# matthewygf/Tiresias

Hardware: AMD Instinct MI355X
Metric: avg JCT + makespan on NSDI'19 Microsoft trace, 8×MI355X cluster (lower is better)
Workload: dtype bf16

## Files before the change

### csrc/bindings/ops.cpp

```cpp
#include <array>
#include <ATen/ATen.h>
#include <c10/hip/HIPStream.h>
#include <torch/library.h>

#include <functional>
#include <map>
#include <mutex>
#include <sstream>
#include <tuple>
#include <vector>

#include "tam/kernels.h"
#include "tam/launch.h"
#include "tam/gemm8p.h"

using at::Tensor;
using c10::optional;

namespace {

hipStream_t cur_stream(const Tensor& t) {
  return c10::hip::getCurrentHIPStream(t.device().index()).stream();
}

// ... 708 lines not shown

void bn_backward_op(const Tensor& dy, const optional<Tensor>& y, const Tensor& x, const Tensor& mean,
                    const Tensor& rstd, const Tensor& gamma, const Tensor& dx,
                    const optional<Tensor>& dres, const optional<Tensor>& dgamma,
                    const optional<Tensor>& dbeta, bool relu, const optional<Tensor>& addend,
                    const optional<Tensor>& sums, bool sums_ready, const optional<Tensor>& ymask) {
  check_bf16(dy, "dy"); check_bf16(x, "x"); check_bf16(dx, "dx");
  check_contig(dy, "dy"); check_contig(x, "x"); check_contig(dx, "dx");
  const int64_t C = x.size(-1);
  const int64_t M = x.numel() / C;
  TORCH_CHECK(C % 8 == 0 && C <= 2048, "tam.bn: C must be a multiple of 8 and <= 2048");
  const bool has_mask = ymask.has_value() && ymask->defined();
  TORCH_CHECK(!relu || (y.has_value() && y->defined()) || has_mask, "tam.bn_backward: relu needs y or ymask");
  if (has_mask)
    TORCH_CHECK(ymask->is_cuda() && ymask->scalar_type() == at::kByte && ymask->is_contiguous() &&
                ymask->numel() == x.numel() / 8, "tam.bn_backward: ymask must be uint8 [numel/8]");
  const tam::bf16_t* yp = has_mask ? nullptr : opt_ptr<const tam::bf16_t>(y);
  const bool has_add = addend.has_value() && addend->defined();
  if (has_add) {
    check_bf16(*addend, "addend"); check_contig(*addend, "addend");
    TORCH_CHECK(addend->numel() == dy.numel(), "tam.bn_backward: addend size");
  }
  TORCH_CHECK(!sums_ready || ((sums.has_value() && sums->defined()) && !relu && !has_add &&
                              !(dres.has_value() && dres->defined())),
              "tam.bn_backward: sums_ready takes the already-masked gradient (no relu / addend / dres)");
  Tensor tmp;
  double* sp = bn_sums(sums, x, C, tmp, "tam.bn_backward");
  tam::bn_backward(bp(dy), opt_ptr<const tam::bf16_t>(addend), yp, bp(x), mean.data_ptr<float>(),
                   rstd.data_ptr<float>(), gamma.data_ptr<float>(), M, (int)C, relu, bpm(dx),
                   opt_ptr<tam::bf16_t>(dres), opt_ptr<float>(dgamma), opt_ptr<float>(dbeta),
                   sp, sums_ready ? 1 : 0, has_mask ? ymask->data_ptr<uint8_t>() : nullptr, cur_stream(x));
}

static tam::LnDrop drop_args(const optional<Tensor>& rec, int64_t site, int64_t thr, double scale,
                             const Tensor& like, const char* op) {
  tam::LnDrop d;
  if (!(rec.has_value() && rec->defined())) return d;
  TORCH_CHECK(rec->scalar_type() == at::kInt && rec->numel() >= 4 && rec->is_contiguous() &&
                  rec->device() == like.device(),
              op, ": drop_rec must be an int32 [4] tensor on the data's device");
  TORCH_CHECK(thr > 0 && thr < 65536 && site >= 0 && site <= 0x7fffffff, op, ": drop_thr in (0, 65536), drop_site >= 0");
  d.rec = rec->data_ptr<int>();
  d.site = (unsigned)site;
  d.thr = (unsigned)thr;
  d.scale = (float)scale;
  return d;
}

void ln_forward_op(const Tensor& x, const Tensor& g, const Tensor& b, const Tensor& y,
                   const Tensor& mean, const Tensor& rstd, double eps, const optional<Tensor>& addend,
                   const optional<Tensor>& sum_out, const optional<Tensor>& drop_rec, int64_t drop_site,
                   int64_t drop_thr, double drop_scale) {
  check_bf16(x, "x"); check_bf16(y, "y"); check_contig(x, "x"); check_contig(y, "y");
  check_f32(g, "g"); check_f32(b, "b");
  const int64_t D = x.size(-1);
  TORCH_CHECK(D % 8 == 0 && D <= 2048, "tam.ln: D must be a multiple of 8 and <= 2048");
  const bool add = addend.has_value() && addend->defined();
  TORCH_CHECK(add == (sum_out.has_value() && sum_out->defined()), "tam.ln_forward: addend needs sum_out");
  if (add) {
    check_bf16(*addend, "addend"); check_contig(*addend, "addend");
    check_bf16(*sum_out, "sum_out"); check_contig(*sum_out, "sum_out");
    TORCH_CHECK(addend->numel() == x.numel() && sum_out->numel() == x.numel(), "tam.ln_forward: addend size");
  }
  const tam::LnDrop drop = drop_args(drop_rec, drop_site, drop_thr, drop_scale, x, "tam.ln_forward");
  TORCH_CHECK(!drop.rec || add, "tam.ln_forward: drop_rec needs addend");
  tam::ln_forward(bp(x), g.data_ptr<float>(), b.data_ptr<float>(), bpm(y), mean.data_ptr<float>(),
// ... 561 lines not shown
                 const optional<Tensor>& dc_next, const optional<Tensor>& dgates,
                 const optional<Tensor>& dc_prev, const optional<Tensor>& dgates_bf16) {
  check_f32(act, "act");
  const int B = (int)act.size(0), Hd = (int)(act.size(1) / 5);
  tam::lstm_cell_backward(act.data_ptr<float>(), opt_ptr<const float>(c_prev), nullptr,
                          opt_ptr<const float>(dh), opt_ptr<const float>(dc_next),
                          opt_ptr<float>(dgates), opt_ptr<float>(dc_prev),
                          opt_ptr<tam::bf16_t>(dgates_bf16), B, Hd, c10::hip::getCurrentHIPStream(act.device().index()).stream());
}

}

TORCH_LIBRARY(tam, m) {
  m.def("gemm(Tensor a, bool a_kmajor, Tensor b, bool b_kmajor, Tensor(a!) c, int mode, Tensor? bias, bool relu, Tensor? mask, float alpha, bool allow_split, Tensor(b!)? colsum=None) -> ()", &gemm_op);
  m.def("conv_fwd(Tensor x, Tensor w, Tensor(a!) y, int stride, int pad, int dil, Tensor? bias, bool relu, Tensor(b!)? stats=None) -> int", &conv_fwd_op);
  m.def("conv_dgrad(Tensor dy, Tensor w, Tensor(a!) wt, Tensor(b!) dx, int stride, int pad, int dil, Tensor? mask) -> ()", &conv_dgrad_op);
  m.def("conv_weight_t_batch(Tensor[] w, Tensor(a!)[] wt) -> ()", &conv_weight_t_batch_op);
  m.def("gemm_wgrad_grouped(Tensor[] dy, Tensor[] x, Tensor(a!)[] dw, Tensor(b!)[] db, int[]? modes=None) -> ()", &gemm_wgrad_grouped_op);
  m.def("gemm_wgrad_grouped_ok(int M, int N, int K) -> bool", &gemm_wgrad_grouped_ok_op);
  m.def("gemm_grouped_tile(int tile) -> ()", &gemm_grouped_tile_op);
  m.def("conv_dgrad_pre(Tensor dy, Tensor w, Tensor wt, Tensor(a!) dx, int stride, int pad, int dil, Tensor? mask, Tensor(b!)? stats=None, Tensor? bnx=None, Tensor? bnmean=None, Tensor? bnrstd=None) -> int", &conv_dgrad_pre_op);
  m.def("conv_wgrad(Tensor dy, Tensor x, Tensor(a!) dw, int stride, int pad, int dil, int mode, Tensor(b!)? dbias=None, bool patch=True) -> ()", &conv_wgrad_op);
  m.def("conv_wgrad_deferred(Tensor dy, Tensor x, Tensor(a!) dw, int stride, int pad, int dil, int mode, Tensor(b!)? dbias, bool patch) -> (Tensor, int)", &conv_wgrad_deferred_op);
  m.def("wgrad_slab_reduce_many(Tensor[] slabs, int[] sp, Tensor(a!)[] dw, int[] mode) -> ()", &wgrad_slab_reduce_many_op);
  m.def("bn_forward(Tensor x, Tensor? res, Tensor(a!) y, Tensor gamma, Tensor beta, Tensor(b!)? run_mean, Tensor(c!)? run_var, Tensor(d!) save_mean, Tensor(e!) save_rstd, float eps, float momentum, bool relu, Tensor(f!)? sums=None, bool sums_ready=False, Tensor(g!)? ymask=None) -> ()", &bn_forward_op);
  m.def("bn_backward(Tensor dy, Tensor? y, Tensor x, Tensor mean, Tensor rstd, Tensor gamma, Tensor(a!) dx, Tensor(b!)? dres, Tensor(c!)? dgamma, Tensor(d!)? dbeta, bool relu, Tensor? addend=None, Tensor(e!)? sums=None, bool sums_ready=False, Tensor? ymask=None) -> ()", &bn_backward_op);
  m.def("ln_forward(Tensor x, Tensor g, Tensor b, Tensor(a!) y, Tensor(b!) mean, Tensor(c!) rstd, float eps, Tensor? addend=None, Tensor(d!)? sum_out=None, Tensor? drop_rec=None, int drop_site=0, int drop_thr=0, float drop_scale=1.0) -> ()", &ln_forward_op);
  m.def("ln_backward(Tensor dy, Tensor x, Tensor g, Tensor mean, Tensor rstd, Tensor(a!) dx, Tensor(b!) dg, Tensor(c!) db, Tensor? addend=None, Tensor(d!)? dr=None, Tensor? drop_rec=None, int drop_site=0, int drop_thr=0, float drop_scale=1.0) -> ()", &ln_backward_op);
  m.def("ln_backward_split(Tensor dy, Tensor x, Tensor g, Tensor mean, Tensor rstd, Tensor(a!) dx, Tensor(b!) ws, Tensor? addend=None, Tensor(c!)? dr=None, Tensor? drop_rec=None, int drop_site=0, int drop_thr=0, float drop_scale=1.0) -> int", &ln_backward_split_op);
  m.def("dropout_apply(Tensor x, Tensor(a!) y, Tensor rec, int site, int thr, float scale) -> ()", &dropout_apply_op);
  m.def("dropout_advance(Tensor(a!) rec) -> ()", &dropout_advance_op);
  m.def("col_reduce_acc(Tensor part, int nblk, int W, Tensor(a!) out0, Tensor(b!) out1, int split) -> ()", &col_reduce_acc_op);
  m.def("col_reduce_acc_batch(Tensor[] parts, int[] nblk, Tensor(a!)[] out0, Tensor(b!)[] out1) -> ()", &col_reduce_acc_batch_op);
  m.def("maxpool_forward(Tensor x, Tensor(a!) y, Tensor(b!) idx, int R, int S, int stride, int pad) -> ()", &maxpool_forward_op);
  m.def("maxpool_backward(Tensor dy, Tensor idx, Tensor(a!) dx, int R, int S, int stride, int pad) -> ()", &maxpool_backward_op);
  m.def("maxpool_k3s2_policy(int policy) -> ()", &maxpool_k3s2_policy_op);
  m.def("avgpool_forward(Tensor x, Tensor(a!) y) -> ()", &avgpool_forward_op);
  m.def("avgpool_backward(Tensor dy, Tensor(a!) dx) -> ()", &avgpool_backward_op);
  m.def("softmax_xent(Tensor logits, Tensor labels, Tensor(a!)? dlogits, Tensor(b!) loss_rows, float smoothing, float grad_scale, int ignore_index, int tm_b=0) -> ()", &softmax_xent_op);
  m.def("embedding_forward(Tensor table, Tensor ids, Tensor(a!) out, float scale, int tm_b=0, Tensor? pos=None) -> ()", &embedding_forward_op);
  m.def("embedding_backward(Tensor dout, Tensor ids, Tensor(a!) gtable, float scale, int tm_b=0) -> ()", &embedding_backward_op);
  m.def("sum_scale(Tensor x, Tensor(a!) out, float scale) -> ()", &sum_scale_op);
  m.def("rows_sum(Tensor[] outs, Tensor[] ins, int[] n_in) -> ()", &rows_sum_op);
  m.def("zero_(Tensor(a!) t) -> ()", &zero_op);
  m.def("colsum(Tensor x, Tensor(a!) out) -> ()", &colsum_op);
  m.def("gemm_force(int cfg, int splits) -> ()", &gemm_force_op);
  m.def("gemm8p_policy(int mode, int tile) -> ()", &gemm8p_policy_op);
  m.def("gemm_pw_policy(int on) -> ()", &gemm_pw_policy_op);
  m.def("conv_pw_gemm_policy(int mode, int tile) -> ()", &conv_pw_gemm_policy_op);
  m.def("policy_names() -> str", &policy_names_op);
  m.def("policy_state() -> int[]", &policy_state_op);
  m.def("policy_load(int[] v) -> ()", &policy_load_op);
  m.def("gemm8p_group(int g) -> ()", &gemm8p_group_op);
  m.def("gemm8p_slab_force(int sp) -> ()", &gemm8p_slab_force_op);
  m.def("gemm_skinny_policy(int on, int force_splits, int nst) -> ()", &gemm_skinny_policy_op);
  m.def("gemm8p_sk_force(int on) -> ()", &gemm8p_sk_force_op);
  m.def("conv_split_policy(int p) -> ()", &conv_split_policy_op);
  m.def("optim_variant(int v) -> ()", &optim_variant_op);
  m.def("optim_grid(int blocks) -> ()", &optim_grid_op);
  m.def("gemm_lib_policy(int policy) -> ()", &gemm_lib_policy_op);
  m.def("conv_dma_policy(int policy) -> ()", &conv_dma_policy_op);
  m.def("conv_wgrad_force(int bm, int bn, int splits, int noatomic=0) -> ()", &conv_wgrad_force_op);
  m.def("conv_wgrad_c64_policy(int policy) -> ()", &conv_wgrad_c64_policy_op);
  m.def("conv_wgrad_order(int flat) -> ()", &conv_wgrad_order_op);
  m.def("conv_stem_policy(int policy) -> ()", &conv_stem_policy_op);
  m.def("conv_wgrad_slab_policy(int policy) -> ()", &conv_wgrad_slab_policy_op);
// ... 31 lines not shown
```

### csrc/include/tam/kernels.h

```cpp
#pragma once
#include <hip/hip_runtime.h>
#include <stdint.h>
#include "tam/common.h"

namespace tam {

constexpr int BN_MAX_BLOCKS = 512;
constexpr int LN_MAX_BLOCKS = 512;
constexpr int COLSUM_MAX_BLOCKS = 256;
void col_reduce_f64(const float* part, int nblk, int W, double* out, hipStream_t s);
constexpr int CR_BATCH_MAX = 48;
void col_reduce_acc_batch(const float* const* part, const int* nblk, const int* W, float* const* out0,
                          float* const* out1, const int* split, int n, hipStream_t s);
void col_reduce_acc(const float* part, int nblk, int W, float* out0, float* out1, int split,
                    hipStream_t s);
void bn_forward(const bf16_t* x, const bf16_t* res, bf16_t* y, long M, int C, float eps,
                float momentum, const float* gamma, const float* beta, float* run_mean,
                float* run_var, float* save_mean, float* save_rstd, int relu, double* sums,
                int sums_ready, uint8_t* ymask, hipStream_t s);
void bn_infer(const bf16_t* x, const bf16_t* res, bf16_t* y, long M, int C, const float* scale,
              const float* shift, int relu, hipStream_t s);
struct WTEntry {
  const bf16_t* w;
  bf16_t* wt;
  int K, RS, C, tile0;
};
constexpr int WT_MAX = 64;
struct WTBatch {
  int n;
  WTEntry e[WT_MAX];
};
void conv_weight_t_batch(WTBatch& b, hipStream_t s);
void bn_backward(const bf16_t* dy, const bf16_t* addend, const bf16_t* y, const bf16_t* x, const float* mean,
                 const float* rstd, const float* gamma, long M, int C, int relu, bf16_t* dx,
                 bf16_t* dres, float* dgamma, float* dbeta, double* sums, int sums_ready,
                 const uint8_t* ymask, hipStream_t s);

struct LnDrop {
  const int* rec = nullptr;
  unsigned site = 0;
  unsigned thr = 0;
  float scale = 1.f;
};
void ln_forward(const bf16_t* x, const float* g, const float* b, bf16_t* y, float* mean,
                float* rstd, long rows, int D, float eps, hipStream_t s, const bf16_t* addend = nullptr,
                bf16_t* sum_out = nullptr, LnDrop drop = {});
void ln_backward(const bf16_t* dy, const bf16_t* x, const float* g, const float* mean,
                 const float* rstd, bf16_t* dx, const bf16_t* addend, float* dg, float* db,
                 float* ws, long rows, int D, hipStream_t s, bf16_t* dres = nullptr, LnDrop drop = {});
int ln_backward_partial(const bf16_t* dy, const bf16_t* x, const float* g, const float* mean,
                        const float* rstd, bf16_t* dx, const bf16_t* addend, float* ws, long rows, int D,
                        hipStream_t s, bf16_t* dres = nullptr, LnDrop drop = {});

void dropout_apply(const bf16_t* x, bf16_t* y, long n, unsigned thr, float scale, const int* rec, int site,
                   hipStream_t s);
void dropout_advance(int* rec, hipStream_t s);

void maxpool_forward(const bf16_t* x, bf16_t* y, uint8_t* idx, int N, int H, int W, int C, int P,
                     int Q, int R, int S, int st, int pad, hipStream_t s);
void maxpool_k3s2_policy(int p);
void maxpool_backward(const bf16_t* dy, const uint8_t* idx, bf16_t* dx, int N, int H, int W, int C,
                      int P, int Q, int R, int S, int st, int pad, hipStream_t s);
void avgpool_forward(const bf16_t* x, bf16_t* y, int N, int HW, int C, hipStream_t s);
void avgpool_backward(const bf16_t* dy, bf16_t* dx, int N, int HW, int C, hipStream_t s);

void softmax_xent(const bf16_t* logits, const long* labels, bf16_t* dlogits, float* loss_rows,
                  long rows, int V, float smoothing, float grad_scale, long ignore_index,
                  hipStream_t s, long tm_b = 0);
void sum_scale(const float* x, long n, float* out, float scale, hipStream_t s);
// ... 86 lines not shown
```

### csrc/kernels/norm.hip

```cpp
#include "tam/common.h"
#include "tam/kernels.h"
#include "tam/philox.h"

namespace tam {

__device__ __forceinline__ void unpack8(const uint4 v, float (&f)[8]) {
  const uint32_t w[4] = {v.x, v.y, v.z, v.w};
#pragma unroll
  for (int i = 0; i < 4; ++i) {
    f[2 * i] = __uint_as_float(w[i] << 16);
    f[2 * i + 1] = __uint_as_float(w[i] & 0xffff0000u);
  }
}
__device__ __forceinline__ uint4 pack8(const float (&f)[8]) {
  return make_uint4(pack_bf2(f[0], f[1]), pack_bf2(f[2], f[3]), pack_bf2(f[4], f[5]),
                    pack_bf2(f[6], f[7]));
}

template <int MODE>
__global__ void __launch_bounds__(256) col_reduce_kernel(const float* __restrict__ part, int nblk,
                                                          int W, double* __restrict__ out64,
                                                          float* __restrict__ out0,
                                                          float* __restrict__ out1, int split) {
  __shared__ double red[16][17];
// ... 510 lines not shown
void bn_infer(const bf16_t* x, const bf16_t* res, bf16_t* y, long M, int C, const float* scale,
              const float* shift, int relu, hipStream_t s) {
  const long total8 = M * C / 8;
  long b = (total8 + 255) / 256;
  if (b > 2048) b = 2048;
  if (b < 1) b = 1;
  hipLaunchKernelGGL(bn_infer_kernel, dim3((unsigned)b), dim3(256), 0, s, x, res, scale, shift, y,
                     total8, C, relu);
}

void bn_backward(const bf16_t* dy, const bf16_t* addend, const bf16_t* y, const bf16_t* x,
                 const float* mean, const float* rstd, const float* gamma, long M, int C, int relu,
                 bf16_t* dx, bf16_t* dres, float* dgamma, float* dbeta, double* sums,
                 int sums_ready, const uint8_t* ymask, hipStream_t s) {
  if (!sums_ready) {
    const BnRed g = bn_reduce_grid(M, C);
    hipLaunchKernelGGL(bn_bwd_reduce_kernel, g.grid, dim3(256), 0, s, dy, addend, y, x, mean, rstd, M,
                       C, g.rows_per_block, g.sw, relu, sums, dres, ymask);
    if (dres) {
      dy = dres;
      addend = nullptr;
      y = nullptr;
      ymask = nullptr;
      relu = 0;
      dres = nullptr;
    }
  }
  const BnGrid g = bn_apply_grid(M, C);
  hipLaunchKernelGGL(bn_bwd_apply_kernel, g.grid, dim3(256), 0, s, dy, addend, y, x, M, C,
                     g.rows_per_block, (const double*)sums, mean, rstd, gamma, dgamma, dbeta, dx, dres,
                     relu, ymask);
}

template <int VEC, bool DROP>
__global__ void __launch_bounds__(256) ln_fwd_kernel(const bf16_t* __restrict__ x,
                                                      const float* __restrict__ g,
                                                      const float* __restrict__ b,
                                                      bf16_t* __restrict__ y,
                                                      float* __restrict__ mean_o,
                                                      float* __restrict__ rstd_o, long rows, int D,
                                                      float eps, const bf16_t* __restrict__ addend,
                                                      bf16_t* __restrict__ sum_out, LnDrop drop) {
  const int lane = threadIdx.x & 63;
  const long row = blockIdx.x * 4L + (threadIdx.x >> 6);
  if (row >= rows) return;
  const bf16_t* xr = x + row * D;
  DropRec dr{};
  if (DROP) dr = DropRec{(uint32_t)drop.rec[0], (uint32_t)drop.rec[1], (uint32_t)drop.rec[2]};
  float f[VEC][8];
  float s = 0.f;
#pragma unroll
  for (int v = 0; v < VEC; ++v) {
    const int c = (v * 64 + lane) * 8;
    if (c < D) {
      unpack8(*(const uint4*)(xr + c), f[v]);
      if (addend) {
        float a[8];
        unpack8(*(const uint4*)(addend + row * D + c), a);
        if (DROP) {
          const uint32_t keep = drop_keep8((uint64_t)(row * D + c) >> 3, drop.site, dr, drop.thr);
#pragma unroll
          for (int j = 0; j < 8; ++j) {
#pragma clang fp contract(off)
            const float t = a[j] * drop.scale;
            if ((keep >> j) & 1u) f[v][j] += t;
          }
// ... 180 lines not shown
```

### tiresias_amd/models/cnn.py

```python
from __future__ import annotations

from typing import List, Tuple

import torch

from ..ops import functional as Fx
from ..ops.arena import Arena


class _BNState:
    def __init__(self, C: int, device):
        self.mean = torch.zeros(C, dtype=torch.float32, device=device)
        self.var = torch.ones(C, dtype=torch.float32, device=device)


class ResNet50:

    name = "resnet50"

    def __init__(self, arena: Arena, num_classes: int = 1000, layers=(3, 4, 6, 3), width: int = 64,
                 in_ch: int = 8):
        self.arena = arena
        dev = arena.device
        self.training = True
# ... 27 lines not shown
                blk["pre"] = pre
                self.blocks.append(blk)
                cin = w * 4
        self.bn_buf, self.bn_ws = Fx.bn_workspaces(
            {k: st.mean.numel() for k, st in self.bn_state.items()}, dev)
        self.fc_w = A.add("fc.w", (num_classes, cin), init="normal", std=0.01)
        self.fc_b = A.add("fc.b", (num_classes,), init="zeros", decay=False)
        self.num_classes = num_classes
        self.in_ch = in_ch

    def _bn(self, x, p, key, relu, res=None, consumer_masks=False):
        st = self.bn_state[key]
        return Fx.batchnorm(x, p[0], p[1], st.mean, st.var, relu=relu, residual=res,
                            training=self.training, consumer_masks=consumer_masks,
                            ws=self.bn_ws[key])

    def _st(self, key):
        return self.bn_ws[key].fwd if (self.training and self.bn_buf.is_cuda) else True

    def conv_params(self):
        out = [self.stem]
        for blk in self.blocks:
            out += [blk["c1"], blk["c2"], blk["c3"]] + ([blk["down"]] if "down" in blk else [])
        return out

    def forward(self, x: torch.Tensor) -> torch.Tensor:
        Fx.prepare_conv_wt(self.conv_params())
        if self.training:
            if self.bn_buf.is_cuda:
                Fx._T().zero_(self.bn_buf)
            else:
                self.bn_buf.zero_()
        y = Fx.conv2d(x, self.stem, stride=2, pad=3, bn_stats=self._st("stem"))
        y = self._bn(y, self.stem_bn, "stem", relu=True)
        y = Fx.maxpool2d(y, 3, 2, 1)
        for blk in self.blocks:
            pre = blk["pre"]
            y, y2 = Fx.residual_split(y)
            idn = y2 if "down" not in blk else None
            o = Fx.conv2d(y, blk["c1"], bn_stats=self._st(pre + ".bn1"))
            o = self._bn(o, blk["bn1"], pre + ".bn1", relu=True, consumer_masks=True)
            o = Fx.conv2d(o, blk["c2"], stride=blk["stride"], pad=1, in_relu=True,
                          bn_stats=self._st(pre + ".bn2"))
            o = self._bn(o, blk["bn2"], pre + ".bn2", relu=True, consumer_masks=True)
            o = Fx.conv2d(o, blk["c3"], in_relu=True, bn_stats=self._st(pre + ".bn3"))
            if "down" in blk:
                idn = Fx.conv2d(y2, blk["down"], stride=blk["stride"],
                                bn_stats=self._st(pre + ".dbn"))
                idn = self._bn(idn, blk["down_bn"], pre + ".dbn", relu=False)
            y = self._bn(o, blk["bn3"], pre + ".bn3", relu=True, res=idn)
        y = Fx.global_avgpool(y)
        return Fx.linear(y, self.fc_w, self.fc_b)

    def buffers(self):
        out = {}
        for k, st in self.bn_state.items():
            out[k + ".mean"] = st.mean
            out[k + ".var"] = st.var
        return out


VGG16_CFG = [64, 64, "M", 128, 128, "M", 256, 256, 256, "M", 512, 512, 512, "M", 512, 512, 512, "M"]


class VGG16:

    name = "vgg16"

# ... 52 lines not shown
```

### tiresias_amd/ops/functional.py

```python
from __future__ import annotations

import math
import os
from typing import List, Optional, Tuple

import torch
import torch.nn.functional as F
from torch.autograd import Function

from . import _lib
from .arena import Param

BF16 = torch.bfloat16


def _T():
    return _lib.ops()


def _cpu_gemm_f32(a: torch.Tensor, b: torch.Tensor) -> torch.Tensor:
    return a.float() @ b.float()


_WGRAD_STREAM = None
# ... 901 lines not shown
        P, Q = _conv_out(H, k, s, p), _conv_out(W, k, s, p)
        if x.is_cuda:
            y = torch.empty(N, P, Q, C, dtype=BF16, device=x.device)
            idx = torch.empty(N, P, Q, C, dtype=torch.uint8, device=x.device)
            _T().maxpool_forward(x, y, idx, k, k, s, p)
            ctx.save_for_backward(idx)
        else:
            y = F.max_pool2d(x.float().permute(0, 3, 1, 2), k, s, p).permute(0, 2, 3, 1).contiguous().to(BF16)
            ctx.save_for_backward(x)
        ctx.cfg = (k, s, p, x.shape)
        return y

    @staticmethod
    def backward(ctx, dy):
        (saved,) = ctx.saved_tensors
        k, s, p, shape = ctx.cfg
        dy = dy.contiguous()
        if dy.is_cuda:
            dx = torch.empty(shape, dtype=BF16, device=dy.device)
            _T().maxpool_backward(dy, saved, dx, k, k, s, p)
        else:
            xf = saved.float().permute(0, 3, 1, 2).requires_grad_(True)
            with torch.enable_grad():
                yf = F.max_pool2d(xf, k, s, p)
                (g,) = torch.autograd.grad(yf, [xf], dy.float().permute(0, 3, 1, 2))
            dx = g.permute(0, 2, 3, 1).contiguous().to(BF16)
        return dx, None, None, None


def maxpool2d(x: torch.Tensor, k: int, s: int, p: int = 0) -> torch.Tensor:
    return _MaxPool.apply(x.contiguous(), k, s, p)


class _AvgPool(Function):
    @staticmethod
    def forward(ctx, x):
        N, H, W, C = x.shape
        if x.is_cuda:
            y = torch.empty(N, C, dtype=BF16, device=x.device)
            _T().avgpool_forward(x, y)
        else:
            y = x.float().mean((1, 2)).to(BF16)
        ctx.shape = x.shape
        return y

    @staticmethod
    def backward(ctx, dy):
        N, H, W, C = ctx.shape
        dy = dy.contiguous()
        if dy.is_cuda:
            dx = torch.empty(ctx.shape, dtype=BF16, device=dy.device)
            _T().avgpool_backward(dy, dx)
        else:
            dx = (dy.float()[:, None, None, :] / (H * W)).expand(N, H, W, C).contiguous().to(BF16)
        return dx


def global_avgpool(x: torch.Tensor) -> torch.Tensor:
    return _AvgPool.apply(x.contiguous())


def softmax_xent(logits: torch.Tensor, labels: torch.Tensor, smoothing: float = 0.0,
                 ignore_index: Optional[int] = -100,
                 normalizer: Optional[int] = None,
                 labels_time_major: bool = False) -> Tuple[torch.Tensor, torch.Tensor]:
    V = logits.shape[-1]
# ... 268 lines not shown
```

Baseline: 0.1231.

## Fuse stem batchnorm, ReLU and 3x3/s2 maxpool into single forward/backward kernels

Adds a fused kernel that applies batchnorm and ReLU to the stem conv output and computes the 3x3 stride-2 maxpool directly, writing only the pooled output, argmax indices and a ReLU bitmask. The goal is to skip materialising the full-resolution post-BN activation and its separate re-read by the pool kernel. The backward path scatters pooled gradients through the saved indices inside the BN reduce and apply kernels, optionally with a second gradient input, instead of running maxpool_backward and then bn_backward. It adds new kernel code, more complex index bookkeeping, and a default policy switch that changes numerics ordering slightly because of bf16 rounding of the gathered gradients.

```diff
diff --git a/csrc/bindings/ops.cpp b/csrc/bindings/ops.cpp
--- a/csrc/bindings/ops.cpp
+++ b/csrc/bindings/ops.cpp
@@ -764,6 +764,64 @@
                    sp, sums_ready ? 1 : 0, has_mask ? ymask->data_ptr<uint8_t>() : nullptr, cur_stream(x));
 }
 
+static void stem_pool_shapes(const Tensor& x, const Tensor& p, const Tensor& idx, const Tensor& ymask,
+                             const char* what) {
+  check_bf16(x, "x"); check_bf16(p, "p"); check_contig(x, "x"); check_contig(p, "p");
+  TORCH_CHECK(x.dim() == 4 && p.dim() == 4, what, ": x and p must be NHWC");
+  const int64_t C = x.size(3);
+  TORCH_CHECK(C % 8 == 0 && C <= 2048, what, ": C must be a multiple of 8 and <= 2048");
+  TORCH_CHECK(x.size(1) >= 1 && x.size(2) >= 1 && x.numel() < (int64_t(1) << 40), what, ": x shape");
+  TORCH_CHECK(p.size(0) == x.size(0) && p.size(1) == (x.size(1) - 1) / 2 + 1 &&
+              p.size(2) == (x.size(2) - 1) / 2 + 1 && p.size(3) == C, what, ": p must be [N][P][Q][C] of the 3x3/s2/p1 pool");
+  TORCH_CHECK(idx.is_cuda() && idx.scalar_type() == at::kByte && idx.is_contiguous() && idx.numel() == p.numel(),
+              what, ": idx must be uint8 with p's element count");
+  TORCH_CHECK(ymask.is_cuda() && ymask.scalar_type() == at::kByte && ymask.is_contiguous() &&
+              ymask.numel() == x.numel() / 8, what, ": ymask must be uint8 [numel/8]");
+}
+
+void bn_relu_maxpool_forward_op(const Tensor& x, const Tensor& p, const Tensor& idx, const Tensor& ymask,
+                                const Tensor& gamma, const Tensor& beta, const optional<Tensor>& run_mean,
+                                const optional<Tensor>& run_var, const Tensor& save_mean,
+                                const Tensor& save_rstd, double eps, double momentum, const Tensor& sums) {
+  stem_pool_shapes(x, p, idx, ymask, "tam.bn_relu_maxpool_forward");
+  check_f32(gamma, "gamma"); check_f32(beta, "beta");
+  const int64_t C = x.size(3);
+  TORCH_CHECK(gamma.numel() == C && beta.numel() == C && save_mean.numel() == C && save_rstd.numel() == C,
+              "tam.bn_relu_maxpool_forward: per-channel tensors must have C elements");
+  Tensor tmp;
+  const double* sp = bn_sums(sums, x, C, tmp, "tam.bn_relu_maxpool_forward");
+  tam::bn_relu_maxpool_forward(bp(x), bpm(p), idx.data_ptr<uint8_t>(), ymask.data_ptr<uint8_t>(),
+                               (int)x.size(0), (int)x.size(1), (int)x.size(2), (int)C, (float)eps,
+                               (float)momentum, gamma.data_ptr<float>(), beta.data_ptr<float>(),
+                               opt_ptr<float>(run_mean), opt_ptr<float>(run_var), save_mean.data_ptr<float>(),
+                               save_rstd.data_ptr<float>(), sp, cur_stream(x));
+}
+
+void bn_relu_maxpool_backward_op(const Tensor& g1, const optional<Tensor>& g2, const Tensor& idx,
+                                 const Tensor& ymask, const Tensor& x, const Tensor& mean, const Tensor& rstd,
+                                 const Tensor& gamma, const Tensor& dx, const optional<Tensor>& dgamma,
+                                 const optional<Tensor>& dbeta, const optional<Tensor>& sums) {
+  stem_pool_shapes(x, g1, idx, ymask, "tam.bn_relu_maxpool_backward");
+  check_bf16(dx, "dx"); check_contig(dx, "dx");
+  TORCH_CHECK(dx.numel() == x.numel(), "tam.bn_relu_maxpool_backward: dx size");
+  const int64_t C = x.size(3);
+  TORCH_CHECK(mean.numel() == C && rstd.numel() == C && gamma.numel() == C,
+              "tam.bn_relu_maxpool_backward: per-channel tensors must have C elements");
+  if (g2.has_value() && g2->defined()) {
+    check_bf16(*g2, "g2"); check_contig(*g2, "g2");
+    TORCH_CHECK(g2->numel() == g1.numel(), "tam.bn_relu_maxpool_backward: g2 size");
+  }
+  Tensor tmp;
+  double* sp = bn_sums(sums, x, C, tmp, "tam.bn_relu_maxpool_backward");
+  tam::bn_relu_maxpool_backward(bp(g1), opt_ptr<const tam::bf16_t>(g2), idx.data_ptr<uint8_t>(),
+                                ymask.data_ptr<uint8_t>(), bp(x), mean.data_ptr<float>(),
+                                rstd.data_ptr<float>(), gamma.data_ptr<float>(), (int)x.size(0),
+                                (int)x.size(1), (int)x.size(2), (int)C, bpm(dx), opt_ptr<float>(dgamma),
+                                opt_ptr<float>(dbeta), sp, cur_stream(x));
+}
+void stem_fuse_policy_op(int64_t p) { tam::stem_fuse_policy((int)p); }
+int64_t stem_fuse_mode_op() { return tam::stem_fuse_mode(); }
+
 static tam::LnDrop drop_args(const optional<Tensor>& rec, int64_t site, int64_t thr, double scale,
                              const Tensor& like, const char* op) {
   tam::LnDrop d;
@@ -1391,6 +1449,10 @@
   m.def("dropout_advance(Tensor(a!) rec) -> ()", &dropout_advance_op);
   m.def("col_reduce_acc(Tensor part, int nblk, int W, Tensor(a!) out0, Tensor(b!) out1, int split) -> ()", &col_reduce_acc_op);
   m.def("col_reduce_acc_batch(Tensor[] parts, int[] nblk, Tensor(a!)[] out0, Tensor(b!)[] out1) -> ()", &col_reduce_acc_batch_op);
+  m.def("bn_relu_maxpool_forward(Tensor x, Tensor(a!) p, Tensor(b!) idx, Tensor(c!) ymask, Tensor gamma, Tensor beta, Tensor(d!)? run_mean, Tensor(e!)? run_var, Tensor(f!) save_mean, Tensor(g!) save_rstd, float eps, float momentum, Tensor sums) -> ()", &bn_relu_maxpool_forward_op);
+  m.def("bn_relu_maxpool_backward(Tensor g1, Tensor? g2, Tensor idx, Tensor ymask, Tensor x, Tensor mean, Tensor rstd, Tensor gamma, Tensor(a!) dx, Tensor(b!)? dgamma, Tensor(c!)? dbeta, Tensor(d!)? sums=None) -> ()", &bn_relu_maxpool_backward_op);
+  m.def("stem_fuse_policy(int policy) -> ()", &stem_fuse_policy_op);
+  m.def("stem_fuse_mode() -> int", &stem_fuse_mode_op);
   m.def("maxpool_forward(Tensor x, Tensor(a!) y, Tensor(b!) idx, int R, int S, int stride, int pad) -> ()", &maxpool_forward_op);
   m.def("maxpool_backward(Tensor dy, Tensor idx, Tensor(a!) dx, int R, int S, int stride, int pad) -> ()", &maxpool_backward_op);
   m.def("maxpool_k3s2_policy(int policy) -> ()", &maxpool_k3s2_policy_op);
diff --git a/csrc/include/tam/kernels.h b/csrc/include/tam/kernels.h
--- a/csrc/include/tam/kernels.h
+++ b/csrc/include/tam/kernels.h
@@ -35,6 +35,16 @@
                  const float* rstd, const float* gamma, long M, int C, int relu, bf16_t* dx,
                  bf16_t* dres, float* dgamma, float* dbeta, double* sums, int sums_ready,
                  const uint8_t* ymask, hipStream_t s);
+void bn_relu_maxpool_forward(const bf16_t* x, bf16_t* p, uint8_t* idx, uint8_t* ymask, int N, int H,
+                             int W, int C, float eps, float momentum, const float* gamma,
+                             const float* beta, float* run_mean, float* run_var, float* save_mean,
+                             float* save_rstd, const double* sums, hipStream_t s);
+void bn_relu_maxpool_backward(const bf16_t* g1, const bf16_t* g2, const uint8_t* idx, const uint8_t* ymask,
+                              const bf16_t* x, const float* mean, const float* rstd, const float* gamma,
+                              int N, int H, int W, int C, bf16_t* dx, float* dgamma, float* dbeta,
+                              double* sums, hipStream_t s);
+void stem_fuse_policy(int p);
+int stem_fuse_mode();
 
 struct LnDrop {
   const int* rec = nullptr;
diff --git a/csrc/kernels/norm.hip b/csrc/kernels/norm.hip
--- a/csrc/kernels/norm.hip
+++ b/csrc/kernels/norm.hip
@@ -566,6 +566,425 @@
                      relu, ymask);
 }
 
+
+static int g_stem_fuse = [] {
+  const char* e = getenv("TAM_STEM_FUSE");
+  return e ? atoi(e) : 1;
+}();
+TAM_KNOB(g_stem_fuse)
+void stem_fuse_policy(int p) { g_stem_fuse = p; }
+int stem_fuse_mode() { return g_stem_fuse; }
+
+static int g_stem_pool_rows = [] {
+  const char* e = getenv("TAM_STEM_POOL_ROWS");
+  return e ? atoi(e) : 4;
+}();
+TAM_KNOB(g_stem_pool_rows)
+
+static int g_stem_bwd_rows = [] {
+  const char* e = getenv("TAM_STEM_BWD_ROWS");
+  return e ? atoi(e) : 2;
+}();
+TAM_KNOB(g_stem_bwd_rows)
+
+__global__ void __launch_bounds__(256) bn_relu_maxpool_fwd_kernel(
+    const bf16_t* __restrict__ x, bf16_t* __restrict__ p, uint8_t* __restrict__ idx,
+    uint8_t* __restrict__ ymask, int N, int H, int W, int C, int P, int Q, int prun, int runs,
+    const double* __restrict__ sums, const float* __restrict__ gamma, const float* __restrict__ beta,
+    float eps, float momentum, float* __restrict__ save_mean, float* __restrict__ save_rstd,
+    float* __restrict__ run_mean, float* __restrict__ run_var) {
+  __shared__ float s_sc[BN_SLAB], s_sh[BN_SLAB];
+  const int c0 = blockIdx.z * BN_SLAB;
+  const int cs = min(BN_SLAB, C - c0);
+  const int t = threadIdx.x;
+  const long M = (long)N * H * W;
+  if (t < cs) {
+    const int c = c0 + t;
+    double S, Qs;
+    bn_shard_sum(sums, C, c, S, Qs);
+    const double mean = S / (double)M;
+    double var = Qs / (double)M - mean * mean;
+    if (var < 0) var = 0;
+    const float rstd = (float)(1.0 / sqrt(var + (double)eps));
+    const float sc = gamma[c] * rstd;
+    s_sc[t] = sc;
+    s_sh[t] = beta[c] - (float)mean * sc;
+    if (blockIdx.x == 0 && blockIdx.y == 0) {
+      save_mean[c] = (float)mean;
+      save_rstd[c] = rstd;
+      if (run_mean) {
+        const double unb = M > 1 ? var * (double)M / (double)(M - 1) : var;
+        run_mean[c] = (1.f - momentum) * run_mean[c] + momentum * (float)mean;
+        run_var[c] = (1.f - momentum) * run_var[c] + momentum * (float)unb;
+      }
+    }
+  }
+  __syncthreads();
+  const int vs = cs / 8;
+  const int e = blockIdx.y * 256 + t;
+  if (e >= Q * vs) return;
+  const int q = e / vs, v = e - q * vs;
+  float sc[8], sh[8];
+#pragma unroll
+  for (int j = 0; j < 8; ++j) { sc[j] = s_sc[v * 8 + j]; sh[j] = s_sh[v * 8 + j]; }
+  const int n = blockIdx.x / runs;
+  const int p0 = (blockIdx.x - n * runs) * prun, p1 = min(P, p0 + prun);
+  const int w0 = 2 * q - 1;
+  const bool in[3] = {w0 >= 0, true, w0 + 2 < W};
+  const long col = c0 + v * 8;
+  const uint4 z = make_uint4(0, 0, 0, 0);
+  auto load = [&](const int h, uint4 (&vx)[3]) {
+    const bf16_t* xr = x + (((long)n * H + h) * W + w0) * C + col;
+#pragma unroll
+    for (int s = 0; s < 3; ++s) vx[s] = in[s] ? *(const uint4*)(xr + (long)s * C) : z;
+  };
+  auto rowbest = [&](const int h, const uint4 (&vx)[3], const bool own, float (&rb)[8], uint32_t (&rs)[8]) {
+#pragma unroll
+    for (int k = 0; k < 8; ++k) { rb[k] = -INFINITY; rs[k] = 0; }
+#pragma unroll
+    for (int s = 0; s < 3; ++s) {
+      if (!in[s]) continue;
+      float f[8];
+      unpack8(vx[s], f);
+#pragma unroll
+      for (int j = 0; j < 8; ++j) {
+        float o = f[j] * sc[j] + sh[j];
+        o = fmaxf(o, 0.f);
+        f[j] = o;
+      }
+      const uint4 pk = pack8(f);
+      const uint32_t wd[4] = {pk.x, pk.y, pk.z, pk.w};
+      if (own && s > 0) {
+        uint32_t bits = 0;
+#pragma unroll
+        for (int k = 0; k < 4; ++k) {
+          bits |= (((wd[k] & 0x8000u) == 0 && (wd[k] & 0x7fffu) != 0) ? 1u : 0u) << (2 * k);
+          bits |= (((wd[k] & 0x80000000u) == 0 && (wd[k] & 0x7fff0000u) != 0) ? 1u : 0u) << (2 * k + 1);
+        }
+        ymask[((((long)n * H + h) * W + w0 + s) * C + col) >> 3] = (uint8_t)bits;
+      }
+#pragma unroll
+      for (int k = 0; k < 4; ++k) {
+        const float a = __uint_as_float(wd[k] << 16), b = __uint_as_float(wd[k] & 0xffff0000u);
+        if (a > rb[2 * k]) { rb[2 * k] = a; rs[2 * k] = s; }
+        if (b > rb[2 * k + 1]) { rb[2 * k + 1] = b; rs[2 * k + 1] = s; }
+      }
+    }
+  };
+  float cb[8];
+  uint32_t ct[8];
+  bool have = false;
+  if (2 * p0 - 1 >= 0) {
+    uint4 vx[3];
+    load(2 * p0 - 1, vx);
+    rowbest(2 * p0 - 1, vx, false, cb, ct);
+    have = true;
+  }
+  for (int pp = p0; pp < p1; ++pp) {
+    const int h1 = 2 * pp, h2 = 2 * pp + 1;
+    const bool has2 = h2 < H;
+    uint4 va[3], vb[3];
+    load(h1, va);
+    if (has2) load(h2, vb);
+    float best[8];
+    uint32_t bi[8];
+#pragma unroll
+    for (int k = 0; k < 8; ++k) { best[k] = -INFINITY; bi[k] = 0; }
+    if (have) {
+#pragma unroll
+      for (int k = 0; k < 8; ++k)
+        if (cb[k] > best[k]) { best[k] = cb[k]; bi[k] = ct[k]; }
+    }
+    {
+      float rb[8];
+      uint32_t rs[8];
+      rowbest(h1, va, true, rb, rs);
+#pragma unroll
+      for (int k = 0; k < 8; ++k)
+        if (rb[k] > best[k]) { best[k] = rb[k]; bi[k] = 3 + rs[k]; }
+    }
+    if (has2) {
+      rowbest(h2, vb, true, cb, ct);
+#pragma unroll
+      for (int k = 0; k < 8; ++k)
+        if (cb[k] > best[k]) { best[k] = cb[k]; bi[k] = 6 + ct[k]; }
+    }
+    have = has2;
+    const long o = (((long)n * P + pp) * Q + q) * C + col;
+    *(uint4*)(p + o) = make_uint4(pack_bf2(best[0], best[1]), pack_bf2(best[2], best[3]),
+                                  pack_bf2(best[4], best[5]), pack_bf2(best[6], best[7]));
+    *(uint2*)(idx + o) = make_uint2(bi[0] | (bi[1] << 8) | (bi[2] << 16) | (bi[3] << 24),
+                                    bi[4] | (bi[5] << 8) | (bi[6] << 16) | (bi[7] << 24));
+  }
+}
+
+void bn_relu_maxpool_forward(const bf16_t* x, bf16_t* p, uint8_t* idx, uint8_t* ymask, int N, int H,
+                             int W, int C, float eps, float momentum, const float* gamma,
+                             const float* beta, float* run_mean, float* run_var, float* save_mean,
+                             float* save_rstd, const double* sums, hipStream_t s) {
+  const int P = (H - 1) / 2 + 1, Q = (W - 1) / 2 + 1;
+  const int prun = g_stem_pool_rows > 0 ? g_stem_pool_rows : 4;
+  const int runs = (P + prun - 1) / prun;
+  const int slabs = (C + BN_SLAB - 1) / BN_SLAB;
+  const int vs = (C < BN_SLAB ? C : BN_SLAB) / 8;
+  const dim3 grid((unsigned)((long)N * runs), (unsigned)((Q * vs + 255) / 256), (unsigned)slabs);
+  hipLaunchKernelGGL(bn_relu_maxpool_fwd_kernel, grid, dim3(256), 0, s, x, p, idx, ymask, N, H, W, C, P,
+                     Q, prun, runs, sums, gamma, beta, eps, momentum, save_mean, save_rstd, run_mean,
+                     run_var);
+}
+
+struct PoolWin {
+  long o[4];
+  uint32_t tap[4];
+};
+__device__ __forceinline__ PoolWin pool_windows(int n, int h, int w, int P, int Q, int C, long col) {
+  const int ps[2] = {(h + 1) >> 1, (h - 1) >> 1}, rs[2] = {(h & 1) ? 0 : 1, 2};
+  const bool pv[2] = {ps[0] < P, (h & 1) != 0};
+  const int qs[2] = {(w + 1) >> 1, (w - 1) >> 1}, ss[2] = {(w & 1) ? 0 : 1, 2};
+  const bool qv[2] = {qs[0] < Q, (w & 1) != 0};
+  PoolWin pw;
+#pragma unroll
+  for (int a = 0; a < 2; ++a)
+#pragma unroll
+    for (int b = 0; b < 2; ++b) {
+      const bool on = pv[a] && qv[b];
+      pw.o[a * 2 + b] = on ? (((long)n * P + ps[a]) * Q + qs[b]) * C + col : 0;
+      pw.tap[a * 2 + b] = on ? (uint32_t)(rs[a] * 3 + ss[b]) : 0xffu;
+    }
+  return pw;
+}
+struct PoolLoad {
+  uint4 g[4], g2[4];
+  uint2 ix[4];
+};
+template <bool TWO>
+__device__ __forceinline__ void pool_load(const PoolWin& pw, const bf16_t* __restrict__ g1,
+                                          const bf16_t* __restrict__ g2, const uint8_t* __restrict__ idx,
+                                          PoolLoad& l) {
+  const uint4 z = make_uint4(0, 0, 0, 0);
+#pragma unroll
+  for (int k = 0; k < 4; ++k) {
+    const bool on = pw.tap[k] != 0xffu;
+    l.ix[k] = on ? *(const uint2*)(idx + pw.o[k]) : make_uint2(0, 0);
+    l.g[k] = on ? *(const uint4*)(g1 + pw.o[k]) : z;
+    if (TWO) l.g2[k] = on ? *(const uint4*)(g2 + pw.o[k]) : z;
+  }
+}
+template <bool TWO>
+__device__ __forceinline__ void pool_gather(const PoolWin& pw, const PoolLoad& l, float (&fd)[8]) {
+  float acc[8] = {0.f, 0.f, 0.f, 0.f, 0.f, 0.f, 0.f, 0.f};
+#pragma unroll
+  for (int k = 0; k < 4; ++k) {
+    if (pw.tap[k] == 0xffu) continue;
+    float d[8];
+    unpack8(l.g[k], d);
+    if (TWO) {
+      float d2[8];
+      unpack8(l.g2[k], d2);
+#pragma unroll
+      for (int i = 0; i < 8; ++i) d[i] += d2[i];
+      unpack8(pack8(d), d);
+    }
+#pragma unroll
+    for (int i = 0; i < 8; ++i) {
+      const uint32_t bb = ((i < 4 ? l.ix[k].x : l.ix[k].y) >> (8 * (i & 3))) & 0xffu;
+      if (bb == pw.tap[k]) acc[i] += d[i];
+    }
+  }
+  unpack8(pack8(acc), fd);
+}
+
+struct Pix {
+  int n, h, w;
+};
+__device__ __forceinline__ Pix pix_of(long r, int H, int W) {
+  const long hw = (long)H * W;
+  const int n = (int)(r / hw);
+  const int rem = (int)(r - (long)n * hw);
+  const int h = rem / W;
+  return Pix{n, h, rem - h * W};
+}
+__device__ __forceinline__ void pix_step(Pix& px, int step, int H, int W) {
+  px.w += step;
+  while (px.w >= W) {
+    px.w -= W;
+    if (++px.h == H) { px.h = 0; ++px.n; }
+  }
+}
+
+template <bool TWO, int U>
+__global__ void __launch_bounds__(256) bn_bwd_reduce_pool_kernel(
+    const bf16_t* __restrict__ g1, const bf16_t* __restrict__ g2, const uint8_t* __restrict__ idx,
+    const uint8_t* __restrict__ ymask, const bf16_t* __restrict__ x, const float* __restrict__ mean,
+    const float* __restrict__ rstd, int H, int W, int P, int Q, long M, int C, long rows_per_block,
+    int sw, double* __restrict__ sums) {
+  __shared__ float red[256 * 16];
+  const int c0 = blockIdx.y * sw;
+  const int cs = min(sw, C - c0);
+  const int tpr = cs / 8, rpb = 256 / tpr;
+  const int cg = threadIdx.x % tpr, rl = threadIdx.x / tpr;
+  const long col = c0 + cg * 8;
+  float a[8], b[8], mu[8], rs[8];
+#pragma unroll
+  for (int i = 0; i < 8; ++i) { a[i] = b[i] = 0.f; mu[i] = mean[col + i]; rs[i] = rstd[col + i]; }
+  const long r0 = blockIdx.x * rows_per_block;
+  const long r1 = min(M, r0 + rows_per_block);
+  auto row = [&](const PoolWin& pw, const PoolLoad& l, const uint4 vx, const uint32_t vm) {
+    float fd[8], fx[8];
+    pool_gather<TWO>(pw, l, fd);
+    unpack8(vx, fx);
+#pragma unroll
+    for (int i = 0; i < 8; ++i) fd[i] = (vm >> i) & 1u ? fd[i] : 0.f;
+#pragma unroll
+    for (int i = 0; i < 8; ++i) {
+      a[i] += fd[i];
+      b[i] += fd[i] * (fx[i] - mu[i]) * rs[i];
+    }
+  };
+  if (rl < rpb && r0 + rl < r1) {
+    long r = r0 + rl;
+    Pix px = pix_of(r, H, W);
+    for (; r + (U - 1) * rpb < r1; r += U * rpb) {
+      PoolWin pw[U];
+      PoolLoad l[U];
+      uint4 vx[U];
+      uint32_t vm[U];
+#pragma unroll
+      for (int u = 0; u < U; ++u) {
+        const long off = (r + u * rpb) * C + col;
+        pw[u] = pool_windows(px.n, px.h, px.w, P, Q, C, col);
+        pool_load<TWO>(pw[u], g1, g2, idx, l[u]);
+        vx[u] = *(const uint4*)(x + off);
+        vm[u] = ymask[off >> 3];
+        pix_step(px, rpb, H, W);
+      }
+#pragma unroll
+      for (int u = 0; u < U; ++u) row(pw[u], l[u], vx[u], vm[u]);
+    }
+    for (; r < r1; r += rpb) {
+      const long off = r * C + col;
+      const PoolWin pw = pool_windows(px.n, px.h, px.w, P, Q, C, col);
+      PoolLoad l;
+      pool_load<TWO>(pw, g1, g2, idx, l);
+      row(pw, l, *(const uint4*)(x + off), ymask[off >> 3]);
+      pix_step(px, rpb, H, W);
+    }
+  }
+#pragma unroll
+  for (int i = 0; i < 8; ++i) { red[threadIdx.x * 16 + i] = a[i]; red[threadIdx.x * 16 + 8 + i] = b[i]; }
+  __syncthreads();
+  if (rl == 0) {
+    for (int j = 1; j < rpb; ++j) {
+      const int t = j * tpr + cg;
+#pragma unroll
+      for (int i = 0; i < 8; ++i) { a[i] += red[t * 16 + i]; b[i] += red[t * 16 + 8 + i]; }
+    }
+  }
+  bn_block_atomics(red, a, b, rl == 0, cg, cs, c0, C, sums);
+}
+
+template <bool TWO, int U>
+__global__ void __launch_bounds__(256) bn_bwd_apply_pool_kernel(
+    const bf16_t* __restrict__ g1, const bf16_t* __restrict__ g2, const uint8_t* __restrict__ idx,
+    const uint8_t* __restrict__ ymask, const bf16_t* __restrict__ x, int H, int W, int P, int Q, long M,
+    int C, long rows_per_block, const double* __restrict__ sums, const float* __restrict__ mean,
+    const float* __restrict__ rstd, const float* __restrict__ gamma, float* __restrict__ dgamma,
+    float* __restrict__ dbeta, bf16_t* __restrict__ dx) {
+  __shared__ float s_k[4][BN_SLAB];
+  const int c0 = blockIdx.y * BN_SLAB;
+  const int cs = min(BN_SLAB, C - c0);
+  const int t = threadIdx.x;
+  if (t < cs) {
+    const int c = c0 + t;
+    double Sd, Qd;
+    bn_shard_sum(sums, C, c, Sd, Qd);
+    const float S = (float)Sd, Qv = (float)Qd;
+    const float rs = rstd[c], gr = gamma[c] * rs;
+    s_k[0][t] = gr;
+    s_k[1][t] = -gr * Qv / (float)M * rs;
+    s_k[2][t] = -gr * S / (float)M;
+    s_k[3][t] = mean[c];
+    if (blockIdx.x == 0) {
+      if (dgamma) dgamma[c] += Qv;
+      if (dbeta) dbeta[c] += S;
+    }
+  }
+  __syncthreads();
+  const int vs = cs / 8, rpp = 256 / vs;
+  const int v = t % vs, rl = t / vs;
+  if (rl >= rpp) return;
+  float k1[8], k2[8], k3[8], mu[8];
+#pragma unroll
+  for (int j = 0; j < 8; ++j) {
+    k1[j] = s_k[0][v * 8 + j]; k2[j] = s_k[1][v * 8 + j]; k3[j] = s_k[2][v * 8 + j]; mu[j] = s_k[3][v * 8 + j];
+  }
+  auto one = [&](const long off, const PoolWin& pw, const PoolLoad& l, const uint4 vx, const uint32_t vm) {
+    float fd[8], fx[8];
+    pool_gather<TWO>(pw, l, fd);
+    unpack8(vx, fx);
+#pragma unroll
+    for (int j = 0; j < 8; ++j) fd[j] = (vm >> j) & 1u ? fd[j] : 0.f;
+    float o[8];
+#pragma unroll
+    for (int j = 0; j < 8; ++j) o[j] = k1[j] * fd[j] + k2[j] * (fx[j] - mu[j]) + k3[j];
+    *(uint4*)(dx + off) = pack8(o);
+  };
+  const long r0 = blockIdx.x * rows_per_block, r1 = min(M, r0 + rows_per_block);
+  const long col = c0 + v * 8;
+  long r = r0 + rl;
+  if (r >= r1) return;
+  Pix px = pix_of(r, H, W);
+  for (; r + (U - 1) * rpp < r1; r += U * rpp) {
+    PoolWin pw[U];
+    PoolLoad l[U];
+    uint4 vx[U];
+    uint32_t vm[U];
+#pragma unroll
+    for (int u = 0; u < U; ++u) {
+      const long off = (r + u * rpp) * C + col;
+      pw[u] = pool_windows(px.n, px.h, px.w, P, Q, C, col);
+      pool_load<TWO>(pw[u], g1, g2, idx, l[u]);
+      vx[u] = *(const uint4*)(x + off);
+      vm[u] = ymask[off >> 3];
+      pix_step(px, rpp, H, W);
+    }
+#pragma unroll
+    for (int u = 0; u < U; ++u) one((r + u * rpp) * C + col, pw[u], l[u], vx[u], vm[u]);
+  }
+  for (; r < r1; r += rpp) {
+    const long off = r * C + col;
+    const PoolWin pw = pool_windows(px.n, px.h, px.w, P, Q, C, col);
+    PoolLoad l;
+    pool_load<TWO>(pw, g1, g2, idx, l);
+    one(off, pw, l, *(const uint4*)(x + off), ymask[off >> 3]);
+    pix_step(px, rpp, H, W);
+  }
+}
+
+void bn_relu_maxpool_backward(const bf16_t* g1, const bf16_t* g2, const uint8_t* idx, const uint8_t* ymask,
+                              const bf16_t* x, const float* mean, const float* rstd, const float* gamma,
+                              int N, int H, int W, int C, bf16_t* dx, float* dgamma, float* dbeta,
+                              double* sums, hipStream_t s) {
+  const int P = (H - 1) / 2 + 1, Q = (W - 1) / 2 + 1;
+  const long M = (long)N * H * W;
+  const BnRed gr = bn_reduce_grid(M, C);
+  const BnGrid ga = bn_apply_grid(M, C);
+  auto launch = [&](auto red, auto app) {
+    hipLaunchKernelGGL(red, gr.grid, dim3(256), 0, s, g1, g2, idx, ymask, x, mean, rstd, H, W, P, Q, M, C,
+                       gr.rows_per_block, gr.sw, sums);
+    hipLaunchKernelGGL(app, ga.grid, dim3(256), 0, s, g1, g2, idx, ymask, x, H, W, P, Q, M, C,
+                       ga.rows_per_block, (const double*)sums, mean, rstd, gamma, dgamma, dbeta, dx);
+  };
+  const bool u2 = g_stem_bwd_rows >= 2;
+  if (g2) {
+    if (u2) launch(bn_bwd_reduce_pool_kernel<true, 2>, bn_bwd_apply_pool_kernel<true, 2>);
+    else launch(bn_bwd_reduce_pool_kernel<true, 1>, bn_bwd_apply_pool_kernel<true, 1>);
+  } else {
+    if (u2) launch(bn_bwd_reduce_pool_kernel<false, 2>, bn_bwd_apply_pool_kernel<false, 2>);
+    else launch(bn_bwd_reduce_pool_kernel<false, 1>, bn_bwd_apply_pool_kernel<false, 1>);
+  }
+}
+
 template <int VEC, bool DROP>
 __global__ void __launch_bounds__(256) ln_fwd_kernel(const bf16_t* __restrict__ x,
                                                       const float* __restrict__ g,
diff --git a/tiresias_amd/models/cnn.py b/tiresias_amd/models/cnn.py
--- a/tiresias_amd/models/cnn.py
+++ b/tiresias_amd/models/cnn.py
@@ -83,8 +83,9 @@
             else:
                 self.bn_buf.zero_()
         y = Fx.conv2d(x, self.stem, stride=2, pad=3, bn_stats=self._st("stem"))
-        y = self._bn(y, self.stem_bn, "stem", relu=True)
-        y = Fx.maxpool2d(y, 3, 2, 1)
+        st = self.bn_state["stem"]
+        y = Fx.stem_bn_pool(y, self.stem_bn[0], self.stem_bn[1], st.mean, st.var,
+                            training=self.training, ws=self.bn_ws["stem"])
         for blk in self.blocks:
             pre = blk["pre"]
             y, y2 = Fx.residual_split(y)
diff --git a/tiresias_amd/ops/functional.py b/tiresias_amd/ops/functional.py
--- a/tiresias_amd/ops/functional.py
+++ b/tiresias_amd/ops/functional.py
@@ -957,6 +957,66 @@
     return _MaxPool.apply(x.contiguous(), k, s, p)
 
 
+class _StemBNPool(Function):
+
+    @staticmethod
+    def forward(ctx, x, token, g: Param, b: Param, run_mean, run_var, eps: float, momentum: float,
+                sums, slot: Optional[GradSlot], ws):
+        N, H, W, C = x.shape
+        P, Q = _conv_out(H, 3, 2, 1), _conv_out(W, 3, 2, 1)
+        p = torch.empty(N, P, Q, C, dtype=BF16, device=x.device)
+        idx = torch.empty(N, P, Q, C, dtype=torch.uint8, device=x.device)
+        ymask = torch.empty(x.numel() // 8, dtype=torch.uint8, device=x.device)
+        mean = torch.empty(C, dtype=torch.float32, device=x.device)
+        rstd = torch.empty_like(mean)
+        _T().bn_relu_maxpool_forward(x, p, idx, ymask, g.master, b.master, run_mean, run_var, mean, rstd,
+                                     eps, momentum, sums)
+        ctx.g, ctx.b, ctx.slot = g, b, slot
+        ctx.bws = ws.bwd if ws is not None else None
+        ctx.save_for_backward(x, idx, ymask, mean, rstd)
+        return p
+
+    @staticmethod
+    def backward(ctx, dp):
+        x, idx, ymask, mean, rstd = ctx.saved_tensors
+        g, b = ctx.g, ctx.b
+        dp = dp.contiguous()
+        dx = torch.empty_like(x)
+        if ctx.slot is not None:
+            add, ctx.slot.stash = ctx.slot.stash, None
+            _T().bn_relu_maxpool_backward(dp, add, idx, ymask, x, mean, rstd, g.master, dx, g.grad, b.grad,
+                                          ctx.bws)
+        else:
+            dy = torch.empty_like(x)
+            _T().maxpool_backward(dp, idx, dy, 3, 3, 2, 1)
+            _T().bn_backward(dy, None, x, mean, rstd, g.master, dx, None, g.grad, b.grad, True, None,
+                             ctx.bws, False, ymask)
+        g.grad_ready()
+        b.grad_ready()
+        return (dx,) + (None,) * 10
+
+
+def stem_fuse_ok(x: torch.Tensor, training: bool) -> bool:
+    return bool(training and x.is_cuda and x.dim() == 4 and x.shape[-1] % 8 == 0
+                and getattr(x, "_tam_bnpart", None) is not None and _T().stem_fuse_mode() != 0)
+
+
+def stem_bn_pool(x: torch.Tensor, g: Param, b: Param, run_mean: Optional[torch.Tensor] = None,
+                 run_var: Optional[torch.Tensor] = None, eps: float = 1e-5, momentum: float = 0.1,
+                 training: bool = True, ws: Optional[BNWorkspace] = None) -> torch.Tensor:
+    if not x.is_contiguous():
+        x = x.contiguous()
+    if not stem_fuse_ok(x, training):
+        y = batchnorm(x, g, b, run_mean, run_var, relu=True, eps=eps, momentum=momentum,
+                      training=training, ws=ws)
+        return maxpool2d(y, 3, 2, 1)
+    slot = GradSlot() if _T().stem_fuse_mode() >= 2 else None
+    p = _StemBNPool.apply(x, g.arena.token, g, b, run_mean, run_var, eps, momentum, x._tam_bnpart, slot, ws)
+    if slot is not None and torch.is_grad_enabled() and p.requires_grad:
+        p._tam_slot = slot
+    return p
+
+
 class _AvgPool(Function):
     @staticmethod
     def forward(ctx, x):
```

New measurement: 0.1238. Within noise of the previous version (+0.6%).
